# pfnet/sfm-learner-chainer

Hardware: AMD Instinct MI355X
Metric: warp+photo-loss fwd+bwd Mpixels/s @128x416x4scales; % HBM roofline (higher is better)
Workload: dtype f32

## Files before the change

### sfm-learner-chainer_amd/csrc/sfm_loss_kernels.h

```cpp
#pragma once
#include "sfm_common.h"
#include "sfm_ssim_pass.h"
#include "sfm_ssim_pair.h"

namespace sfm {

constexpr int MAX_CHUNK_ROWS = 28;
constexpr int MIN_CHUNK_ROWS = 4;
constexpr int WAVES_PER_BLOCK = 1;

struct ScaleArgs {
  const float* tgt;
  const float* src;
  const float* disp;
  const float* mlog;
  float* d_disp;
  float* d_mask;
  float* d_src;
  float* warped;
  int h, w, strips, chunks, tiles, item_begin, chunk_rows;
  float inv_cnt;
  float c_dx2, c_dy2, c_dxy;
  float c_ex, c_ey;
  float c_exp;
// ... 24 lines not shown
  Base = 0,
  Wide = 1,
  Pair = 2,
  Ref = 3,
  Dsrc = 4,
};
struct Variant {
  bool grad, loss;
  bool ssim, expl;
  int smode;
  bool hwc, warped;
  Family family;
};

struct HaloCols { int hs, hm, hr, hl, sw; };
constexpr HaloCols halo_of(const bool ssim, const bool grad, const int smode) {
  const int hs = ssim ? (grad ? 2 : 1) : 0;
  const int hm = smode == 1 ? 2 : (smode == 2 ? 1 : 0);
  const int hr = hs > hm ? hs : hm;
  const int hl = grad ? hr : hs;
  return {hs, hm, hr, hl, 64 - hl - hr};
}
constexpr HaloCols halo_of(const Variant& v) { return halo_of(v.ssim, v.grad, v.smode); }
template <bool SSIM, bool GRAD, int SMODE>
struct Halo {
  static constexpr int HS = halo_of(SSIM, GRAD, SMODE).hs, HR = halo_of(SSIM, GRAD, SMODE).hr, HL = halo_of(SSIM, GRAD, SMODE).hl,
                       SW = halo_of(SSIM, GRAD, SMODE).sw;
};
constexpr int waves_per_simd(const Family f, const bool ssim, const bool grad) {
  return f == Family::Pair ? 2 : (f == Family::Wide || (ssim && grad)) ? 3 : 4;
}
constexpr int waves_per_simd(const Variant& v) { return waves_per_simd(v.family, v.ssim, v.grad); }
constexpr int sources_per_pass(const Family f) { return f == Family::Pair ? 2 : 1; }

__device__ __forceinline__ void tile_put(float* p, const float v, const bool add) {
  if (add) *p = *p + v;
  else *p = v;
}

template <bool GRAD, bool LOSS>
__device__ __forceinline__ void smooth2_pass(const LossArgs& A, const ScaleArgs& S, const float* __restrict__ dplane, int lane,
                                             int x, bool xin, bool outl, int y0, int y1, float* gacc, float& acc_sm, const bool add) {
  const int h = S.h, w = S.w;
  const bool vx2 = xin && (x <= w - 3);
  const bool vx1 = xin && (x <= w - 2);
  const unsigned xc = (unsigned)min(max(x, 0), w - 1);
  auto ldrow = [&](int r) -> float { return ldf(dplane, (unsigned)min(max(r, 0), h - 1) * (unsigned)w + xc); };
  float c_dx2 = S.c_dx2, c_dy2 = S.c_dy2, c_dxy = S.c_dxy, gyv = A.gy;
  asm volatile("" : "+v"(c_dx2), "+v"(c_dy2), "+v"(c_dxy), "+v"(gyv));
  float s2y_m1 = 0.f, s2y_m2 = 0.f, txy_m1 = 0.f;
  auto row = [&](const int a, float& d0, float& dp1, float& q) {
    q = xin ? q : 0.f;
    const float dp2 = q;
    const float dxr0 = from_right(d0) - d0;
    const float dx2 = from_right(dxr0) - dxr0;
    const float dy0 = dp1 - d0, dy1 = dp2 - dp1;
    const float dy2 = dy1 - dy0;
    const float dxrp = from_right(dp1) - dp1;
    const float dxdy0 = dxrp - dxr0;
    const float dydx0 = from_right(dy0) - dy0;
    d0 = ldrow(a + 5);
    const bool va = a >= 0, va2 = va && a <= h - 3, va1 = va && a <= h - 2;
    if (LOSS) {
      if (a >= y0) {
        float t = 0.f;
        if (vx2) t += c_dx2 * fabsf(dx2);
// ... 209 lines not shown
  const int prio_rank = min((int)(blockIdx.x >> 3) / H.simds_per_xcd, H.prio_top);
  set_issue_prio((int)((H.prio_tab >> (2 * prio_rank)) & 3u));
  const int chunk = t / S.strips;
  const int strip = t - chunk * S.strips;
  const int h = S.h, w = S.w;
  const int lane = threadIdx.x & 63;
  const int x = strip * HH::SW - HH::HL + lane;
  const bool xin = (x >= 0) && (x < w);
  const bool outl = (lane >= HH::HL) && (lane < 64 - HH::HR) && (x < w);
  const int y0 = chunk * S.chunk_rows;
  const int y1 = min(y0 + S.chunk_rows, h);
  const ScaleConst sc = make_scale_const(h, w);
  const size_t P = (size_t)h * w;

  float acc_pix = 0.f, acc_ssim = 0.f, acc_sm = 0.f, acc_exp = 0.f;
  bool first = true;
  float disp_first, disp_second;
  {
    const float* dpl = S.disp + (size_t)b * P;
    const int rfirst = y0 - HH::HS;
    const unsigned xcl = (unsigned)min(max(x, 0), w - 1);
    disp_first = ldf(dpl, (unsigned)min(max(rfirst, 0), h - 1) * (unsigned)w + xcl);
    disp_second = ldf(dpl, (unsigned)min(max(rfirst + 1, 0), h - 1) * (unsigned)w + xcl);
  }
  static_assert(SFM_MAX_SRC * 8 <= 64, "one group of eight lanes per source");
  WaveGeom WG;
  WaveGeomRef WGR;
  build_wave_geom_any<REF != 0>(A.pose, H.n_src, b, A.intrinsics + (size_t)(b * H.n_scales + s) * 9, lane, WG, WGR);
#ifdef SFM_STAMPS
  Stamps st = {0, 0, 0, 0, 0};
  unsigned long long ts0 = 0, cyc_smooth = 0, cyc_src = 0;
  SFM_STAMP(ts0);
#endif
  const bool smooth_last = (SMODE != 0) && (prio_rank == 1);
  const int n_units = PAIR ? (H.n_src >> 1) : H.n_src;
  const int n_phases = n_units + (SMODE != 0 ? 1 : 0);
  for (int ph = 0; ph < n_phases; ++ph) {
    const int iu = (SMODE != 0 && !smooth_last) ? ph - 1 : ph;
    const int i = PAIR ? 2 * iu : iu;
#ifdef SFM_STAMPS
    unsigned long long tp0 = 0, tp1 = 0;
    SFM_STAMP(tp0);
#endif
    if (SMODE != 0 && (iu < 0 || iu >= n_units)) {
      if (SMODE == 1) smooth2_pass<GRAD, LOSS>(A, S, S.disp + (size_t)b * P, lane, x, xin, outl, y0, y1, gacc, acc_sm, !first);
      else smooth_edge_pass<GRAD, LOSS, HWC>(A, S, S.disp + (size_t)b * P, S.tgt + (size_t)b * 3 * P, lane, x, xin, outl, y0, y1, gacc, acc_sm, !first);
      first = false;
#ifdef SFM_STAMPS
      SFM_STAMP(tp1);
      cyc_smooth += tp1 - tp0;
#endif
      continue;
    }
    if (iu * 2 >= n_units) set_issue_prio((int)((H.prio_tab >> (8 + 2 * prio_rank)) & 3u));
    SsimCtx C;
    const float xf = (float)x;
    C.x0 = x - lane;
    if constexpr (REF != 0) {
#pragma unroll
      for (int k = 0; k < 3; ++k) {
        C.Pm[k * 4 + 0] = from_lane(WGR.P0, 8 * i + k);
        C.Pm[k * 4 + 1] = from_lane(WGR.P1, 8 * i + k);
        C.Pm[k * 4 + 2] = from_lane(WGR.P2, 8 * i + k);
        C.Pm[k * 4 + 3] = from_lane(WGR.P3, 8 * i + k);
        C.Ki1[k] = from_lane(WGR.Ki1, k);
        C.Ki2[k] = from_lane(WGR.Ki2, k);
        C.mx[k] = from_lane(WGR.Ki0, k) * xf;
        C.M1[k] = C.P3[k] = 0.f;
      }
#pragma unroll
      for (int k = 0; k < 3; ++k) C.P3[k] = C.Pm[k * 4 + 3];
      C.hw[0] = 0.5f * sc.wm1; C.hw[1] = 0.5f * sc.hm1;
      C.rhw[0] = uniform(rcp_refined(C.hw[0])); C.rhw[1] = uniform(rcp_refined(C.hw[1]));
    } else {
#pragma unroll
      for (int k = 0; k < 3; ++k) {
        C.M1[k] = from_lane(WG.M1, 8 * i + k);
        C.P3[k] = from_lane(WG.P3, 8 * i + k);
        C.mx[k] = fmaf(from_lane(WG.M0, 8 * i + k), xf, from_lane(WG.M2, 8 * i + k));
      }
    }
#pragma unroll
    for (int k = 0; k < 3; ++k) {
      C.tp[k] = S.tgt + ((size_t)b * 3 + k) * P;
      C.sp[k] = S.src + (((size_t)b * H.n_src + i) * 3 + k) * P;
    }
    C.k_pix = S.k_pix;
    C.kq = S.kq;
    C.k_exp = S.k_exp;
    int y0p = y0, y1p = y1;
    asm volatile("" : "+s"(y0p), "+s"(y1p));
    C.h = h; C.w = w; C.y0 = y0p; C.y1 = y1p;
    C.dp = S.disp + (size_t)b * P;
    C.dsp = (DSRC && S.d_src) ? S.d_src + ((size_t)b * H.n_src + i) * 3 * P : nullptr;
    C.wp = WARPED ? S.warped + ((size_t)b * H.n_src + i) * 3 * P : nullptr;
    C.mp = EXPL ? S.mlog + ((size_t)b * H.n_src + i) * P : nullptr;
    C.dmp = (EXPL && GRAD) ? S.d_mask + ((size_t)b * H.n_src + i) * P : nullptr;
    C.P = P;
    C.sc = sc;
    C.xc = (unsigned)min(max(x, 0), w - 1);
    C.disp_first = disp_first;
    C.disp_second = disp_second;
    C.xc12 = 12u * C.xc;
    C.x12 = 12u * (unsigned)x;
    C.img12 = 12u * (unsigned)h * (unsigned)w;
    C.w12 = 12u * (unsigned)w;
    C.w12f = (float)(12 * w);
    C.xin = xin;
    C.outb = outl;
    C.xinf = xin ? 1.f : 0.f;
    C.outf = outl ? 1.f : 0.f;
    C.lane = lane;
    float* gpm_out = GRAD ? A.part_gpm + ((size_t)item * H.n_src + i) * 12 : nullptr;
    if constexpr (PAIR) {
      SsimCtx Cb = C;
#pragma unroll
      for (int k = 0; k < 3; ++k) {
        Cb.M1[k] = from_lane(WG.M1, 8 * (i + 1) + k);
        Cb.P3[k] = from_lane(WG.P3, 8 * (i + 1) + k);
        Cb.mx[k] = fmaf(from_lane(WG.M0, 8 * (i + 1) + k), xf, from_lane(WG.M2, 8 * (i + 1) + k));
        Cb.sp[k] = C.sp[k] + 3 * P;
      }
      Cb.wp = WARPED ? C.wp + 3 * P : nullptr;
      ssim_pair_pass<GRAD, LOSS, WARPED>(C, Cb, gacc, first, acc_pix, acc_ssim, gpm_out, GRAD ? gpm_out + 12 : nullptr);
    } else if constexpr (SSIM) {
      ssim_source_pass<GRAD, LOSS, HWC, WARPED, REF, DSRC>(C, gacc, first, acc_pix, acc_ssim, gpm_out SFM_STAMPS_PASS);
    } else {
      l1_source_pass<GRAD, LOSS, EXPL, HWC, WARPED, REF, DSRC>(C, gacc, first, acc_pix, acc_exp, gpm_out);
    }
    first = false;
#ifdef SFM_STAMPS
    SFM_STAMP(tp1);
    cyc_src += tp1 - tp0;
#endif
  }
  if (LOSS) {
    float v[4] = {acc_pix, acc_ssim, acc_sm, acc_exp};
    wave_sums_lockstep(v);
    if (lane == 63) {
      float* o = A.part_loss + (size_t)item * 4;
      o[0] = v[0] * S.inv_cnt; o[1] = v[1] * S.inv_cnt; o[2] = v[2]; o[3] = v[3] * S.c_exp;
    }
  }
  if (GRAD) {
    if (outl) {
      float* o = S.d_disp + (size_t)b * P;
      for (int q = y0; q < y1; ++q) stf_wt(o, (unsigned)(q * w + x), gacc[(q - y0) * 64 + lane]);
    }
  }
  if (H.trace && lane == 0) {
    unsigned long long* o = H.trace + (size_t)item * 4;
    o[0] = t_start;
    o[1] = __builtin_amdgcn_s_memrealtime();
    o[2] = __builtin_amdgcn_s_getreg((4) | (0 << 6) | (31 << 11));
    o[3] = (__builtin_amdgcn_s_getreg((20) | (0 << 6) | (31 << 11)) & 0xf) | ((unsigned long long)blockIdx.x << 8);
#ifdef SFM_STAMPS
    {
      unsigned long long* q = H.trace + (size_t)H.items * 4 + (size_t)item * 8;
      unsigned long long ts3 = 0;
      SFM_STAMP(ts3);
      q[0] = st.a_fin; q[1] = st.a_iss; q[2] = st.b; q[3] = st.c; q[4] = st.steps > 0 ? st.steps : 1;
      q[5] = cyc_smooth;
      q[6] = cyc_src;
      q[7] = ts3 - ts0;
    }
#endif
  }
}

template <bool SSIM, bool GRAD, bool LOSS, bool EXPL, int SMODE, bool HWC, bool WARPED = false>
__global__ void __launch_bounds__(64 * WAVES_PER_BLOCK, waves_per_simd(Family::Base, SSIM, GRAD)) loss_kernel(SFM_HDR_PARAMS, const LossArgs A) {
  loss_body<SSIM, GRAD, LOSS, EXPL, SMODE, HWC, WARPED>(make_hdr(A, SFM_HDR_ARGS), A);
}
template <bool SSIM, bool LOSS, bool EXPL, int SMODE, bool HWC, bool WARPED = false>
__global__ void __launch_bounds__(64 * WAVES_PER_BLOCK, waves_per_simd(Family::Dsrc, SSIM, true)) loss_kernel_dsrc(SFM_HDR_PARAMS, const LossArgs A) {
  loss_body<SSIM, true, LOSS, EXPL, SMODE, HWC, WARPED, 0, true>(make_hdr(A, SFM_HDR_ARGS), A);
}
template <bool SSIM, bool GRAD, bool LOSS, bool EXPL, int SMODE, bool HWC, bool WARPED = false>
__global__ void __launch_bounds__(64 * WAVES_PER_BLOCK, waves_per_simd(Family::Ref, SSIM, GRAD)) loss_kernel_ref(SFM_HDR_PARAMS, const LossArgs A) {
  loss_body<SSIM, GRAD, LOSS, EXPL, SMODE, HWC, WARPED, 1, GRAD>(make_hdr(A, SFM_HDR_ARGS), A);
}
template <bool GRAD, bool LOSS, int SMODE>
__global__ void __launch_bounds__(64 * WAVES_PER_BLOCK, waves_per_simd(Family::Pair, true, GRAD)) loss_kernel_pair(SFM_HDR_PARAMS, const LossArgs A) {
  loss_body<true, GRAD, LOSS, false, SMODE, true, false, 0, false, true>(make_hdr(A, SFM_HDR_ARGS), A);
}
template <bool LOSS, int SMODE, bool HWC, bool WARPED = false>
__global__ void __launch_bounds__(64 * WAVES_PER_BLOCK, waves_per_simd(Family::Wide, false, true)) loss_kernel_wide(SFM_HDR_PARAMS, const LossArgs A) {
  loss_body<false, true, LOSS, false, SMODE, HWC, WARPED>(make_hdr(A, SFM_HDR_ARGS), A);
}

template <Family F, bool GRAD, bool LOSS, bool SSIM, bool EXPL, int SMODE, bool HWC, bool WARPED>
const void* family_kernel() {
  if constexpr (F == Family::Base) return (const void*)&loss_kernel<SSIM, GRAD, LOSS, EXPL, SMODE, HWC, WARPED>;
  else if constexpr (F == Family::Ref) return (const void*)&loss_kernel_ref<SSIM, GRAD, LOSS, EXPL, SMODE, HWC, WARPED>;
  else if constexpr (F == Family::Dsrc && GRAD) return (const void*)&loss_kernel_dsrc<SSIM, LOSS, EXPL, SMODE, HWC, WARPED>;
// ... 66 lines not shown
```

### sfm-learner-chainer_amd/csrc/sfm_ssim_pass.h

```cpp
#pragma once
#include "sfm_common.h"

namespace sfm {

#ifdef SFM_STAMPS
#define SFM_STAMP(var) do { __builtin_amdgcn_sched_barrier(0); asm volatile("s_memtime %0\n s_waitcnt lgkmcnt(0)" : "=s"(var) :: "memory"); __builtin_amdgcn_sched_barrier(0); } while (0)
struct Stamps { unsigned long long a_fin, a_iss, b, c, steps; };
static __device__ Stamps g_dummy_stamps;
#define SFM_STAMPS_ARG , Stamps& st
#define SFM_STAMPS_PASS , st
#else
#define SFM_STAMP(var) do { } while (0)
#define SFM_STAMPS_ARG
#define SFM_STAMPS_PASS
#endif

struct SsimCtx {
  float M1[3], P3[3];
  float Ki1[3], Ki2[3], Pm[12], hw[2], rhw[2];
  int x0;
  float k_pix;
  float kq;
  int h, w, y0, y1;
  const float* tp[3];
  const float* sp[3];
  const float* dp;
  float* dsp;
  float* wp;
  const float* mp;
  float* dmp;
  float k_exp;
  size_t P;
  ScaleConst sc;
  float mx[3];
  float disp_first, disp_second;
  unsigned xc;
  unsigned xc12;
  unsigned x12;
  unsigned img12;
  unsigned w12;
  float w12f;
  bool xin;
  bool outb;
  float xinf;
  float outf;
  int lane;
};

typedef float f2 __attribute__((ext_vector_type(2)));
struct Ch3 {
  f2 p;
  float s;
};
__device__ __forceinline__ Ch3 ch3(float c0, float c1, float c2) { Ch3 r; r.p.x = c0; r.p.y = c1; r.s = c2; return r; }
__device__ __forceinline__ Ch3 ch3_zero() { return ch3(0.f, 0.f, 0.f); }

template <typename T> __device__ __forceinline__ T T_of(float v);
template <> __device__ __forceinline__ float T_of<float>(float v) { return v; }
template <> __device__ __forceinline__ f2 T_of<f2>(float v) { f2 r; r.x = v; r.y = v; return r; }
__device__ __forceinline__ f2 vfma(f2 a, f2 b, f2 c) { return __builtin_elementwise_fma(a, b, c); }
__device__ __forceinline__ float vfma(float a, float b, float c) { return fmaf(a, b, c); }
__device__ __forceinline__ f2 vrcp(f2 a) { f2 r; r.x = rcp(a.x); r.y = rcp(a.y); return r; }
__device__ __forceinline__ float vrcp(float a) { return rcp(a); }
__device__ __forceinline__ f2 hsum3(f2 v) { f2 r; r.x = hsum3(v.x); r.y = hsum3(v.y); return r; }
// ... 30 lines not shown
}
__device__ __forceinline__ void hsum3_group(f2& a, f2& b, f2& c, float& e, float& f, float& g) {
  pin(a); pin(b); pin(c); pin(e); pin(f); pin(g);
  __builtin_amdgcn_sched_barrier(0);
  const float le = add_left(e), lf = add_left(f), lg = add_left(g);
  const f2 la = add_left(a), lb = add_left(b), lc = add_left(c);
  e = add_right(le, e); f = add_right(lf, f); g = add_right(lg, g);
  a = add_right(la, a); b = add_right(lb, b); c = add_right(lc, c);
  __builtin_amdgcn_sched_barrier(0);
}
__device__ __forceinline__ float half_one_minus_clamped(float S) { return fminf(fmaxf(fmaf(S, -0.5f, 0.5f), 0.f), 1.f); }
__device__ __forceinline__ f2 half_one_minus_clamped(f2 S) {
  f2 r;
  asm("v_pk_fma_f32 %0, %1, 0.5, 0.5 op_sel_hi:[1,0,0] neg_lo:[1,0,0] neg_hi:[1,0,0] clamp" : "=v"(r) : "v"(S));
  return r;
}
__device__ __forceinline__ float sign01(float d) {
  const float big = 0x1p127f;
  float sp, sm;
  asm("v_mul_f32_e64 %0, %1, %2 clamp" : "=v"(sp) : "v"(d), "s"(big));
  asm("v_mul_f32_e64 %0, -%1, %2 clamp" : "=v"(sm) : "v"(d), "s"(big));
  return sp - sm;
}
__device__ __forceinline__ f2 sign01(f2 d) {
  f2 big;
  big.x = 0x1p127f; big.y = 0x1p127f;
  f2 sp, sm;
  asm("v_pk_mul_f32 %0, %1, %2 clamp" : "=v"(sp) : "v"(d), "s"(big));
  asm("v_pk_mul_f32 %0, %1, %2 neg_lo:[1,0] neg_hi:[1,0] clamp" : "=v"(sm) : "v"(d), "s"(big));
  return sp - sm;
}
__device__ __forceinline__ float ksign(float k, float d) { return k * sign01(d); }
__device__ __forceinline__ f2 ksign(float k, f2 d) { return sign01(d) * k; }
__device__ __forceinline__ float add_ksign(float g, float k, float d) { return fmaf(sign01(d), k, g); }
__device__ __forceinline__ f2 add_ksign(f2 g, float k, f2 d) { return vfma(sign01(d), T_of<f2>(k), g); }
__device__ __forceinline__ float vabs_sum(f2 d) { return fabsf(d.x) + fabsf(d.y); }
__device__ __forceinline__ float vabs_sum(float d) { return fabsf(d); }
__device__ __forceinline__ float vhadd(f2 v) { return v.x + v.y; }
__device__ __forceinline__ float vhadd(float v) { return v; }

struct __attribute__((packed, aligned(4))) Rgb {
  float c[3];
};
__device__ __forceinline__ Rgb load_rgb(const float* p) { return *reinterpret_cast<const Rgb*>(p); }
struct __attribute__((packed, aligned(4))) K9 {
  float k[9];
};
__device__ __forceinline__ K9 load_k9(const float* Kp) { return *reinterpret_cast<const K9*>(Kp); }

__device__ __forceinline__ float from_lane(const float v, const int k) {
  return __builtin_bit_cast(float, __builtin_amdgcn_readlane(__builtin_bit_cast(int, v), k));
}
__device__ __forceinline__ float from_lane_v(const float v, const int src) {
  return __builtin_bit_cast(float, __builtin_amdgcn_ds_bpermute(src << 2, __builtin_bit_cast(int, v)));
}

__device__ __forceinline__ void inv3_fast(const float* K, float* o) {
  const float a = K[0], b = K[1], c = K[2], d = K[3], e = K[4], f = K[5], g = K[6], h = K[7], i = K[8];
  const float A = fmaf(e, i, -(f * h)), B = fmaf(f, g, -(d * i)), Cc = fmaf(d, h, -(e * g));
  const float det = fmaf(a, A, fmaf(b, B, c * Cc));
  const float r = rcp_refined(det);
  o[0] = A * r;
  o[1] = fmaf(c, h, -(b * i)) * r;
  o[2] = fmaf(b, f, -(c * e)) * r;
  o[3] = B * r;
  o[4] = fmaf(a, i, -(c * g)) * r;
// ... 102 lines not shown
  f2 duv0, duv1, duv_s;
  f2 UV;
  float D;
  float rzi;
  float nm;
};
struct RowG { Ch3 a, b, e; };

struct Pipe {
  float ta[3], tb[3];
  float ba[3], bb[3];
  float it[3];
  f2 UV, f;
  float rz, D;
  float lg;
  bool inview;
  bool inview_o;
};

__device__ __forceinline__ void zero(RowS& s) {
  s.ih = s.it = ch3_zero(); s.duv0 = s.duv1 = s.duv_s = T_of<f2>(0.f);
  s.UV = T_of<f2>(0.f); s.D = s.rzi = s.nm = 0.f;
}
__device__ __forceinline__ void zero(RowG& s) { s.a = s.b = s.e = ch3_zero(); }
__device__ __forceinline__ float opaque_zero() {
  float z;
  asm volatile("v_mov_b32 %0, 0" : "=v"(z));
  return z;
}
__device__ __forceinline__ Ch3 ch3_opaque_zero() {
  const float a = opaque_zero(), b = opaque_zero(), c = opaque_zero();
  return ch3(a, b, c);
}
__device__ __forceinline__ void zero_rare(RowS& s) {
  s.ih = ch3_opaque_zero(); s.it = ch3_opaque_zero();
  s.duv0.x = opaque_zero(); s.duv0.y = opaque_zero(); s.duv1.x = opaque_zero(); s.duv1.y = opaque_zero(); s.duv_s.x = opaque_zero(); s.duv_s.y = opaque_zero();
  s.UV.x = opaque_zero(); s.UV.y = opaque_zero(); s.D = opaque_zero(); s.rzi = opaque_zero(); s.nm = opaque_zero();
}

struct __attribute__((packed, aligned(4))) Rgb2 {
  float c[6];
};

struct RefPos {
  f2 UV;
  f2 fr, cell;
  float rz, D;
  bool inview;
};
__device__ __forceinline__ Proj ref_proj_cell(const RefPos& rp, const int h, const int w) {
  Proj p;
  p.U = rp.UV.x; p.V = rp.UV.y; p.rz = rp.rz; p.inview = rp.inview;
  int u0 = (int)rp.cell.x, v0 = (int)rp.cell.y;
  p.fu = rp.fr.x; p.fv = rp.fr.y;
  if (u0 > w - 2) { u0 = w - 2; p.fu = 1.f; }
  if (v0 > h - 2) { v0 = h - 2; p.fv = 1.f; }
  p.u0 = rp.inview ? u0 : 0;
  p.v0 = rp.inview ? v0 : 0;
  return p;
}
__device__ __forceinline__ RefPos ref_position(const SsimCtx& C, const float yf, const float D ) {
  RefPos o;
  o.D = D;
  f2 ray, q, kxp, Ki1p, Ki2p, Pc0, Pc1, Pc2, Pc3, hwp, rhwp, whm1;
  kxp.x = C.mx[0]; kxp.y = C.mx[1]; Ki1p.x = C.Ki1[0]; Ki1p.y = C.Ki1[1]; Ki2p.x = C.Ki2[0]; Ki2p.y = C.Ki2[1];
  Pc0.x = C.Pm[0]; Pc0.y = C.Pm[4]; Pc1.x = C.Pm[1]; Pc1.y = C.Pm[5]; Pc2.x = C.Pm[2]; Pc2.y = C.Pm[6]; Pc3.x = C.Pm[3]; Pc3.y = C.Pm[7];
  hwp.x = C.hw[0]; hwp.y = C.hw[1]; rhwp.x = C.rhw[0]; rhwp.y = C.rhw[1]; whm1.x = C.sc.wm1; whm1.y = C.sc.hm1;
  float q2;
  {
#pragma clang fp contract(off)
    ray = (kxp + Ki1p * yf) + Ki2p;
    const float ray2 = (C.mx[2] + C.Ki1[2] * yf) + C.Ki2[2];
    const f2 c = ray * o.D;
    const float c2 = ray2 * o.D;
    q = ((Pc0 * c.x + Pc1 * c.y) + Pc2 * c2) + Pc3;
    q2 = ((C.Pm[8] * c.x + C.Pm[9] * c.y) + C.Pm[10] * c2) + C.Pm[11];
  }
  const float z = q2 + 1e-10f;
  o.rz = rcp(z);
  const f2 qr = q * o.rz;
  o.UV = vfma(vfma(-qr, T_of<f2>(z), q), T_of<f2>(o.rz), qr);
  const f2 xr = o.UV * rhwp;
  const f2 xn = vfma(vfma(-xr, hwp, o.UV), rhwp, xr) - 1.0f;
  const f2 t = vfma(-xn, xn, T_of<f2>(1.0f));
  o.inview = (t.x > 0.0f) & (t.y > 0.0f);
  f2 up;
  {
#pragma clang fp contract(off)
    up = ((xn + 1.0f) * whm1) * 0.5f + 1.0f;
  }
  o.fr.x = __builtin_amdgcn_fractf(up.x); o.fr.y = __builtin_amdgcn_fractf(up.y);
  o.cell = (up - o.fr) - 1.0f;
  return o;
}

template <bool HWC, int REF = 0, bool SECOND = false>
__device__ __forceinline__ void issue_row(const SsimCtx& C, const int r, const float disp, Pipe& ps) {
  static_assert(!SECOND || (HWC && REF == 0), "two sources per pass: pixel-interleaved layout, the product's projection");
  const float yf = (float)r;
  Proj p;
  f2 UV, fr, cell;
  float rz;
  if constexpr (REF != 0) {
    const RefPos rp = ref_position(C, yf, rcp_refined(disp));
    ps.D = rp.D; UV = rp.UV; fr = rp.fr; cell = rp.cell; rz = rp.rz; p.inview = rp.inview;
    p.u0 = p.v0 = 0;
    if constexpr (!HWC) {
      p = ref_proj_cell(rp, C.h, C.w);
      fr.x = p.fu; fr.y = p.fv;
    }
  } else if constexpr (HWC) {
    if constexpr (!SECOND) ps.D = rcp(disp);
    f2 M1p, mxp, P3p, whm1;
    M1p.x = C.M1[0]; M1p.y = C.M1[1]; mxp.x = C.mx[0]; mxp.y = C.mx[1]; P3p.x = C.P3[0]; P3p.y = C.P3[1];
    whm1.x = C.sc.wm1; whm1.y = C.sc.hm1;
    const f2 a = vfma(M1p, T_of<f2>(yf), mxp);
    const float a2 = fmaf(C.M1[2], yf, C.mx[2]);
    const f2 q = vfma(T_of<f2>(ps.D), a, P3p);
    const float z = fmaf(ps.D, a2, C.P3[2]) + 1e-10f;
    rz = rcp(z);
    const f2 qr = q * rz;
    UV = vfma(vfma(-qr, T_of<f2>(z), q), T_of<f2>(rz), qr);
    const f2 sg = UV * (whm1 - UV);
    p.inview = (sg.x > 0.0f) & (sg.y > 0.0f);
    fr.x = __builtin_amdgcn_fractf(UV.x); fr.y = __builtin_amdgcn_fractf(UV.y);
    cell = UV - fr;
    p.u0 = p.v0 = 0;
  } else {
    ps.D = rcp(disp);
    const float a0 = fmaf(C.M1[0], yf, C.mx[0]), a1 = fmaf(C.M1[1], yf, C.mx[1]), a2 = fmaf(C.M1[2], yf, C.mx[2]);
    p = project(a0, a1, a2, C.P3[0], C.P3[1], C.P3[2], ps.D, C.sc, C.h, C.w);
    UV.x = p.U; UV.y = p.V; fr.x = p.fu; fr.y = p.fv; rz = p.rz;
    cell = UV;
  }
  ps.UV = UV; ps.f = fr;
  if constexpr (HWC) {
    ps.rz = (p.inview && C.outb) ? rz : 0.f;
    ps.inview = ps.inview_o = true;
  } else {
    ps.rz = rz;
    ps.inview = p.inview && C.xin;
    ps.inview_o = p.inview && C.outb;
  }
  const unsigned off = (unsigned)(p.v0 * C.w + p.u0);
  const unsigned offt = (unsigned)r * (unsigned)C.w + C.xc;
  if constexpr (HWC) {
    const float bof = fmaf(cell.y, C.w12f, cell.x * 12.f);
    const char* sp8 = reinterpret_cast<const char*>(C.sp[0]);
    const char* tp8 = reinterpret_cast<const char*>(C.tp[0]) + (size_t)((unsigned)r * C.w12);
    const __amdgpu_buffer_rsrc_t srs = __builtin_amdgcn_make_buffer_rsrc(const_cast<char*>(sp8), 0, (int)C.img12, 0x00027000);
    const __amdgpu_buffer_rsrc_t srs2 = __builtin_amdgcn_make_buffer_rsrc(const_cast<char*>(sp8 + C.w12), 0, (int)(C.img12 - C.w12), 0x00027000);
    const __amdgpu_buffer_rsrc_t trs = __builtin_amdgcn_make_buffer_rsrc(const_cast<char*>(tp8), 0, (int)C.w12, 0x00027000);
    const unsigned o12 = (p.inview && C.xin) ? (unsigned)bof : 0x80000000u;
    typedef unsigned u4v __attribute__((ext_vector_type(4)));
    typedef unsigned u3v __attribute__((ext_vector_type(3)));
    typedef unsigned u2v __attribute__((ext_vector_type(2)));
    const u4v t0 = __builtin_amdgcn_raw_buffer_load_b128(srs, o12, 0, 0);
    const u2v t1 = __builtin_amdgcn_raw_buffer_load_b64(srs, o12 + 16u, 0, 0);
    const u4v b0 = __builtin_amdgcn_raw_buffer_load_b128(srs2, o12, 0, 0);
    const u2v b1 = __builtin_amdgcn_raw_buffer_load_b64(srs2, o12 + 16u, 0, 0);
    u3v i0 = {0u, 0u, 0u};
    if constexpr (!SECOND) i0 = __builtin_amdgcn_raw_buffer_load_b96(trs, C.x12, 0, 0);
    Rgb2 T, Bt;
    Rgb I;
// ... 46 lines not shown
  }
}

__device__ __forceinline__ void store_warped_row(const SsimCtx& C, const int r, const RowS& s) {
  if ((unsigned)(r - C.y0) < (unsigned)(C.y1 - C.y0) && C.outb) {
    const unsigned o = (unsigned)r * (unsigned)C.w + C.xc;
    stf_wt(C.wp, o, s.ih.p.x);
    stf_wt(C.wp + C.P, o, s.ih.p.y);
    stf_wt(C.wp + 2 * C.P, o, s.ih.s);
  }
}

struct PoseAcc {
  f2 A, B, Cq;
  float A2, B2, C2;
};
__device__ __forceinline__ void zero(PoseAcc& a) {
  a.A = a.B = a.Cq = T_of<f2>(0.f); a.A2 = a.B2 = a.C2 = 0.f;
}


__device__ __forceinline__ float geom_terms(const SsimCtx& C, const f2 UV, const float D, const float yf, const f2 gq, PoseAcc& gpm) {
  const f2 guv = gq * UV;
  const float gq2 = -(guv.x + guv.y);
  const f2 t = gq * D;
  const float t2 = gq2 * D;
  const float gdisp = fmaf(t.x, C.P3[0], fmaf(t.y, C.P3[1], t2 * C.P3[2]));
  gpm.A += t; gpm.A2 += t2;
  gpm.B = vfma(T_of<f2>(yf), t, gpm.B); gpm.B2 = fmaf(yf, t2, gpm.B2);
  gpm.Cq += gq; gpm.C2 += gq2;
  return gdisp;
}

template <bool DSRC , int REF = 0>
__device__ __forceinline__ void geometry_backward(const SsimCtx& C, const RowS& s2, const int rc, const f2 gq,
                                                  const float* gI, float* gacc, const bool first, PoseAcc& gpm) {
  const int h = C.h, w = C.w;
  const float yf = (float)rc;
  const float gdisp = geom_terms(C, s2.UV, s2.D, yf, gq, gpm);
  float* ga = gacc + (rc - C.y0) * 64 + C.lane;
  if (first) *ga = gdisp;
  else *ga = *ga + gdisp;
  if (DSRC && C.dsp != nullptr && C.outb) {
    struct __attribute__((packed, aligned(4))) Rec { float c[3]; };
    const unsigned o = (unsigned)rc * (unsigned)w + (unsigned)(C.x0 + C.lane);
    Rec g; g.c[0] = gI[0]; g.c[1] = gI[1]; g.c[2] = gI[2];
    reinterpret_cast<Rec*>(C.dsp)[o] = g;
  }
  (void)h;
}

__device__ __forceinline__ void pose_sums_raw(const SsimCtx& C, const PoseAcc& pa, float* gpm_out) {
  const float acc[9] = {pa.A.x, pa.A.y, pa.A2, pa.B.x, pa.B.y, pa.B2, pa.Cq.x, pa.Cq.y, pa.C2};
  const float xf = (float)(C.x0 + C.lane);
  float v[12];
#pragma unroll
  for (int k = 0; k < 3; ++k) {
    v[k * 4 + 0] = xf * acc[k];
    v[k * 4 + 1] = acc[3 + k];
    v[k * 4 + 2] = acc[k];
    v[k * 4 + 3] = acc[6 + k];
  }
  wave_sums_lockstep(v);
  if (C.lane == 63) {
    float4* o = reinterpret_cast<float4*>(gpm_out);
    o[0] = make_float4(v[0], v[1], v[2], v[3]);
    o[1] = make_float4(v[4], v[5], v[6], v[7]);
    o[2] = make_float4(v[8], v[9], v[10], v[11]);
  }
}

template <typename T>
struct SsimSums { T Sx, Sy, Sqq, Sxy; };

template <typename T>
// ... 44 lines not shown
  g = add_ksign(vfma(vfma(it, Eq, -(ih * Bq)), T_of<T>(9.f), Aq), kpn, diff);
}

template <bool GRAD, bool LOSS>
__device__ __forceinline__ void ssim_stage_b_row(const SsimCtx& C, const RowS& s2, const RowS& s1, const RowS& s0, RowG& g0,
                                                 const bool count, float& acc_pix, float& acc_ssim) {
  float ssum = 0.f;
  const float kq2_nm = C.kq * s1.nm;
  SsimSums<f2> pp;
  SsimSums<float> ps;
  ssim_vsums(s2.ih.p, s1.ih.p, s0.ih.p, s2.it.p, s1.it.p, s0.it.p, pp);
  ssim_vsums(s2.ih.s, s1.ih.s, s0.ih.s, s2.it.s, s1.it.s, s0.it.s, ps);
  hsum3_group(pp.Sx, pp.Sy, pp.Sqq, pp.Sxy, ps.Sx, ps.Sy, ps.Sqq, ps.Sxy);
  ssim_value_partials<GRAD, LOSS, true>(pp, kq2_nm, g0.a.p, g0.b.p, g0.e.p, ssum);
  ssim_value_partials<GRAD, LOSS, false>(ps, kq2_nm, g0.a.s, g0.b.s, g0.e.s, ssum);
  if (GRAD) hsum3_group(g0.a.p, g0.b.p, g0.e.p, g0.a.s, g0.b.s, g0.e.s);
  if (LOSS) {
    const float wgt = count ? s1.nm * C.outf : 0.f;
    acc_ssim = fmaf(ssum, wgt, acc_ssim);
    if (!GRAD) {
      const float e1 = vabs_sum(s1.ih.p - s1.it.p) + vabs_sum(s1.ih.s - s1.it.s);
      acc_pix = fmaf(e1, wgt, acc_pix);
    }
  }
}

__device__ __forceinline__ f2 contract_uv(const RowS& s, const f2 gp, const float gs) {
  f2 hq = T_of<f2>(gp.x) * s.duv0;
  hq = vfma(T_of<f2>(gp.y), s.duv1, hq);
  hq = vfma(T_of<f2>(gs), s.duv_s, hq);
  return hq * s.rzi;
}

template <bool LOSS, bool DSRC, int REF = 0>
__device__ __forceinline__ void ssim_stage_c_row(const SsimCtx& C, const int rc, const RowS& s2, const RowG& g2, const RowG& g1,
                                                 const RowG& g0, float* gacc, const bool first, PoseAcc& gpm, float& acc_pix) {
  const float kpn = C.k_pix * s2.nm;
  f2 gp, dp;
  float gs, ds;
  ssim_stage_c(g2.a.p, g1.a.p, g0.a.p, g2.b.p, g1.b.p, g0.b.p, g2.e.p, g1.e.p, g0.e.p, s2.ih.p, s2.it.p, kpn, gp, dp);
  ssim_stage_c(g2.a.s, g1.a.s, g0.a.s, g2.b.s, g1.b.s, g0.b.s, g2.e.s, g1.e.s, g0.e.s, s2.ih.s, s2.it.s, kpn, gs, ds);
  if (LOSS) acc_pix = fmaf(vabs_sum(dp) + vabs_sum(ds), s2.nm * C.outf, acc_pix);
  const float gI[3] = {gp.x, gp.y, gs};
  geometry_backward<DSRC, REF>(C, s2, rc, contract_uv(s2, gp, gs), gI, gacc, first, gpm);
}

struct StepMasks {
  unsigned fin;
  unsigned iss;
  unsigned b;
  unsigned cnt;
  unsigned c;
};
__device__ __forceinline__ unsigned step_range(int lo, int hi) {
  lo = min(max(lo, 0), 32);
  hi = min(max(hi, lo), 32);
  const unsigned long long one = 1ull;
  return (unsigned)(((one << hi) - 1ull) & ~((one << lo) - 1ull));
}
__device__ __forceinline__ bool step_bit(const unsigned m, const int k) { return ((m >> k) & 1u) != 0u; }

template <bool GRAD, bool LOSS, bool HWC, bool WARPED, int REF, bool DSRC>
__device__ __forceinline__ void ssim_row_step(const SsimCtx& C, const StepMasks& M, const int k, const int r, Pipe& ps, float& disp_next,
                                              RowS& s0, const RowS& s1, const RowS& s2,
                                              RowG& g0, const RowG& g1, const RowG& g2, float* gacc, const bool first,
                                              float& acc_pix, float& acc_ssim, PoseAcc& gpm SFM_STAMPS_ARG) {
  const int w = C.w;
#ifdef SFM_STAMPS
  unsigned long long t0 = 0, t1 = 0, t2 = 0, t3 = 0, t4 = 0;
#endif
  SFM_STAMP(t0);
  finish_row<HWC>(C, ps, s0);
  if (!step_bit(M.fin, k)) zero_rare(s0);
  if constexpr (WARPED) store_warped_row(C, r, s0);
  SFM_STAMP(t1);
  if (step_bit(M.iss, k)) {
    issue_row<HWC, REF>(C, r + 1, disp_next, ps);
    disp_next = ldf(C.dp, (unsigned)min(r + 2, C.h - 1) * (unsigned)w + C.xc);
  }
  SFM_STAMP(t2);

  if (step_bit(M.b, k)) {
    ssim_stage_b_row<GRAD, LOSS>(C, s2, s1, s0, g0, step_bit(M.cnt, k), acc_pix, acc_ssim);
  }

  SFM_STAMP(t3);
  if (GRAD) {
    if (step_bit(M.c, k)) {
      ssim_stage_c_row<LOSS, DSRC, REF>(C, r - 2, s2, g2, g1, g0, gacc, first, gpm, acc_pix);
    }
  }
  SFM_STAMP(t4);
#ifdef SFM_STAMPS
  st.a_fin += t1 - t0; st.a_iss += t2 - t1; st.b += t3 - t2; st.c += t4 - t3; st.steps += 1;
#endif
}

template <bool GRAD, bool LOSS, bool HWC, bool WARPED, int REF = 0, bool DSRC = false>
__device__ __forceinline__ void ssim_source_pass(const SsimCtx& C, float* gacc, const bool first, float& acc_pix, float& acc_ssim,
                                                 float* gpm_out  SFM_STAMPS_ARG) {
  constexpr int HS = GRAD ? 2 : 1;
  const int rbeg = C.y0 - HS, rend = C.y1 + HS;
  const int rload = min(rend, C.h);
  PoseAcc gpm;
  zero(gpm);
  RowS S0, S1, S2;
  RowG G0, G1, G2;
  Pipe ps;
  float disp_next = 1.f;
  const int n = rend - rbeg, R = C.y1 - C.y0;
  StepMasks M;
  M.fin = step_range(-rbeg, C.h - rbeg);
  M.iss = step_range(-rbeg - 1, rload - rbeg - 1);
  M.b = step_range(HS + 1 - (GRAD ? 1 : 0), n);
  M.cnt = step_range(HS + 1, HS + 1 + R);
  M.c = step_range(HS + 2, HS + 2 + R);
  if (rbeg >= 0 && rbeg < C.h) issue_row<HWC, REF>(C, rbeg, C.disp_first, ps);
  disp_next = C.disp_second;
  for (int k = 0; k < n; k += 3) {
    const int r = rbeg + k;
    ssim_row_step<GRAD, LOSS, HWC, WARPED, REF, DSRC>(C, M, k, r, ps, disp_next, S0, S2, S1, G0, G2, G1, gacc, first, acc_pix, acc_ssim, gpm SFM_STAMPS_PASS);
    if (k + 1 < n)
      ssim_row_step<GRAD, LOSS, HWC, WARPED, REF, DSRC>(C, M, k + 1, r + 1, ps, disp_next, S1, S0, S2, G1, G0, G2, gacc, first, acc_pix, acc_ssim, gpm SFM_STAMPS_PASS);
    if (k + 2 < n)
      ssim_row_step<GRAD, LOSS, HWC, WARPED, REF, DSRC>(C, M, k + 2, r + 2, ps, disp_next, S2, S1, S0, G2, G1, G0, gacc, first, acc_pix, acc_ssim, gpm SFM_STAMPS_PASS);
  }
  if (GRAD) {
    pose_sums_raw(C, gpm, gpm_out);
  }
}

template <bool GRAD, bool LOSS, bool EXPL, bool HWC, bool WARPED, int REF = 0, bool DSRC = false>
__device__ __forceinline__ void l1_source_pass(const SsimCtx& C, float* gacc, const bool first, float& acc_pix, float& acc_exp,
                                               float* gpm_out) {
  PoseAcc gpm;
  zero(gpm);
  Pipe ps;
  ps.lg = 0.f;
  float disp_next = 1.f;
  const int rbeg = C.y0, rend = C.y1;
  issue_row<HWC, REF>(C, rbeg, C.disp_first, ps);
  if (rbeg + 1 < rend) disp_next = C.disp_second;
  for (int r = rbeg; r < rend; ++r) {
    RowS s0;
    finish_row<HWC>(C, ps, s0);
    if constexpr (WARPED) store_warped_row(C, r, s0);
    const float lg = ps.lg;
    if (r + 1 < rend) issue_row<HWC, REF>(C, r + 1, disp_next, ps);
    disp_next = ldf(C.dp, (unsigned)min(r + 2, C.h - 1) * (unsigned)C.w + C.xc);
    float sgm = 1.f;
    if (EXPL) {
      sgm = rcp(1.0f + __expf(-lg));
      if (LOSS) acc_exp += C.outf * (fmaxf(-lg, 0.f) + __logf(1.0f + __expf(-fabsf(lg))));
    }
    const float e1 = (vabs_sum(s0.ih.p - s0.it.p) + vabs_sum(s0.ih.s - s0.it.s)) * s0.nm;
    if (LOSS) acc_pix = fmaf(e1 * sgm, C.outf, acc_pix);
    if (GRAD) {
      const float kpn = C.k_pix * s0.nm * sgm;
// ... 16 lines not shown
```

Before: 80990.

## Fuse edge-aware smoothness pass into the first or last SSIM source pass

When SSIM with edge-aware smoothness is active (non-pair, not ref-grad), the separate smoothness phase is removed. The smoothness loss and gradient are computed inside an SSIM source pass, reusing the target rows and disparity already loaded there. On the last source, the disparity gradient is combined with the pending geometry gradient before being stored. This removes one full pass over the disparity and target planes per tile. In exchange, the fused variant keeps raw disparity in the row state and recomputes its reciprocal in the backward step, which adds register pressure and arithmetic.

Result: slower. 78650 (-2.9%).

```diff
diff --git a/sfm-learner-chainer_amd/csrc/sfm_loss_kernels.h b/sfm-learner-chainer_amd/csrc/sfm_loss_kernels.h
--- a/sfm-learner-chainer_amd/csrc/sfm_loss_kernels.h
+++ b/sfm-learner-chainer_amd/csrc/sfm_loss_kernels.h
@@ -80,6 +80,7 @@
 }
 constexpr int waves_per_simd(const Variant& v) { return waves_per_simd(v.family, v.ssim, v.grad); }
 constexpr int sources_per_pass(const Family f) { return f == Family::Pair ? 2 : 1; }
+constexpr bool fuse_smooth(const bool ssim, const int smode, const bool pair, const bool ref_grad) { return ssim && smode == 2 && !pair && !ref_grad; }
 
 __device__ __forceinline__ void tile_put(float* p, const float v, const bool add) {
   if (add) *p = *p + v;
@@ -355,17 +356,18 @@
   unsigned long long ts0 = 0, cyc_smooth = 0, cyc_src = 0;
   SFM_STAMP(ts0);
 #endif
+  constexpr bool FUSED = fuse_smooth(SSIM, SMODE, PAIR, REF != 0 && GRAD);
   const bool smooth_last = (SMODE != 0) && (prio_rank == 1);
   const int n_units = PAIR ? (H.n_src >> 1) : H.n_src;
-  const int n_phases = n_units + (SMODE != 0 ? 1 : 0);
+  const int n_phases = n_units + ((SMODE != 0 && !FUSED) ? 1 : 0);
   for (int ph = 0; ph < n_phases; ++ph) {
-    const int iu = (SMODE != 0 && !smooth_last) ? ph - 1 : ph;
+    const int iu = (SMODE != 0 && !FUSED && !smooth_last) ? ph - 1 : ph;
     const int i = PAIR ? 2 * iu : iu;
 #ifdef SFM_STAMPS
     unsigned long long tp0 = 0, tp1 = 0;
     SFM_STAMP(tp0);
 #endif
-    if (SMODE != 0 && (iu < 0 || iu >= n_units)) {
+    if (SMODE != 0 && !FUSED && (iu < 0 || iu >= n_units)) {
       if (SMODE == 1) smooth2_pass<GRAD, LOSS>(A, S, S.disp + (size_t)b * P, lane, x, xin, outl, y0, y1, gacc, acc_sm, !first);
       else smooth_edge_pass<GRAD, LOSS, HWC>(A, S, S.disp + (size_t)b * P, S.tgt + (size_t)b * 3 * P, lane, x, xin, outl, y0, y1, gacc, acc_sm, !first);
       first = false;
@@ -411,6 +413,10 @@
     C.k_pix = S.k_pix;
     C.kq = S.kq;
     C.k_exp = S.k_exp;
+    if constexpr (FUSED) {
+      C.cex = S.c_ex; C.cey = S.c_ey;
+      C.gcx = uniform(A.gy * S.c_ex); C.gcy = uniform(A.gy * S.c_ey);
+    }
     int y0p = y0, y1p = y1;
     asm volatile("" : "+s"(y0p), "+s"(y1p));
     C.h = h; C.w = w; C.y0 = y0p; C.y1 = y1p;
@@ -446,8 +452,16 @@
       }
       Cb.wp = WARPED ? C.wp + 3 * P : nullptr;
       ssim_pair_pass<GRAD, LOSS, WARPED>(C, Cb, gacc, first, acc_pix, acc_ssim, gpm_out, GRAD ? gpm_out + 12 : nullptr);
+    } else if constexpr (FUSED) {
+      if (GRAD && smooth_last) {
+        if (iu == n_units - 1) ssim_source_pass<GRAD, LOSS, HWC, WARPED, REF, DSRC, GRAD ? 2 : 1, true>(C, gacc, first, acc_pix, acc_ssim, acc_sm, gpm_out SFM_STAMPS_PASS);
+        else ssim_source_pass<GRAD, LOSS, HWC, WARPED, REF, DSRC, 0, true>(C, gacc, first, acc_pix, acc_ssim, acc_sm, gpm_out SFM_STAMPS_PASS);
+      } else {
+        if (iu == 0) ssim_source_pass<GRAD, LOSS, HWC, WARPED, REF, DSRC, 1, true>(C, gacc, first, acc_pix, acc_ssim, acc_sm, gpm_out SFM_STAMPS_PASS);
+        else ssim_source_pass<GRAD, LOSS, HWC, WARPED, REF, DSRC, 0, true>(C, gacc, first, acc_pix, acc_ssim, acc_sm, gpm_out SFM_STAMPS_PASS);
+      }
     } else if constexpr (SSIM) {
-      ssim_source_pass<GRAD, LOSS, HWC, WARPED, REF, DSRC>(C, gacc, first, acc_pix, acc_ssim, gpm_out SFM_STAMPS_PASS);
+      ssim_source_pass<GRAD, LOSS, HWC, WARPED, REF, DSRC>(C, gacc, first, acc_pix, acc_ssim, acc_sm, gpm_out SFM_STAMPS_PASS);
     } else {
       l1_source_pass<GRAD, LOSS, EXPL, HWC, WARPED, REF, DSRC>(C, gacc, first, acc_pix, acc_exp, gpm_out);
     }
@@ -483,7 +497,7 @@
       unsigned long long ts3 = 0;
       SFM_STAMP(ts3);
       q[0] = st.a_fin; q[1] = st.a_iss; q[2] = st.b; q[3] = st.c; q[4] = st.steps > 0 ? st.steps : 1;
-      q[5] = cyc_smooth;
+      q[5] = FUSED ? (1ull << 63) | st.sm : cyc_smooth;
       q[6] = cyc_src;
       q[7] = ts3 - ts0;
     }
diff --git a/sfm-learner-chainer_amd/csrc/sfm_ssim_pass.h b/sfm-learner-chainer_amd/csrc/sfm_ssim_pass.h
--- a/sfm-learner-chainer_amd/csrc/sfm_ssim_pass.h
+++ b/sfm-learner-chainer_amd/csrc/sfm_ssim_pass.h
@@ -5,7 +5,7 @@
 
 #ifdef SFM_STAMPS
 #define SFM_STAMP(var) do { __builtin_amdgcn_sched_barrier(0); asm volatile("s_memtime %0\n s_waitcnt lgkmcnt(0)" : "=s"(var) :: "memory"); __builtin_amdgcn_sched_barrier(0); } while (0)
-struct Stamps { unsigned long long a_fin, a_iss, b, c, steps; };
+struct Stamps { unsigned long long a_fin, a_iss, b, c, steps, sm; };
 static __device__ Stamps g_dummy_stamps;
 #define SFM_STAMPS_ARG , Stamps& st
 #define SFM_STAMPS_PASS , st
@@ -30,6 +30,7 @@
   const float* mp;
   float* dmp;
   float k_exp;
+  float cex, cey, gcx, gcy;
   size_t P;
   ScaleConst sc;
   float mx[3];
@@ -126,6 +127,7 @@
 }
 __device__ __forceinline__ float ksign(float k, float d) { return k * sign01(d); }
 __device__ __forceinline__ f2 ksign(float k, f2 d) { return sign01(d) * k; }
+__device__ __forceinline__ float ksign_med3(float k, float d) { return k * __builtin_amdgcn_fmed3f(d * 0x1p127f, -1.f, 1.f); }
 __device__ __forceinline__ float add_ksign(float g, float k, float d) { return fmaf(sign01(d), k, g); }
 __device__ __forceinline__ f2 add_ksign(f2 g, float k, f2 d) { return vfma(sign01(d), T_of<f2>(k), g); }
 __device__ __forceinline__ float vabs_sum(f2 d) { return fabsf(d.x) + fabsf(d.y); }
@@ -294,10 +296,12 @@
   const float a = opaque_zero(), b = opaque_zero(), c = opaque_zero();
   return ch3(a, b, c);
 }
+template <bool KEEP_D = false>
 __device__ __forceinline__ void zero_rare(RowS& s) {
   s.ih = ch3_opaque_zero(); s.it = ch3_opaque_zero();
   s.duv0.x = opaque_zero(); s.duv0.y = opaque_zero(); s.duv1.x = opaque_zero(); s.duv1.y = opaque_zero(); s.duv_s.x = opaque_zero(); s.duv_s.y = opaque_zero();
-  s.UV.x = opaque_zero(); s.UV.y = opaque_zero(); s.D = opaque_zero(); s.rzi = opaque_zero(); s.nm = opaque_zero();
+  s.UV.x = opaque_zero(); s.UV.y = opaque_zero(); s.rzi = opaque_zero(); s.nm = opaque_zero();
+  if constexpr (!KEEP_D) s.D = opaque_zero();
 }
 
 struct __attribute__((packed, aligned(4))) Rgb2 {
@@ -356,30 +360,32 @@
   return o;
 }
 
-template <bool HWC, int REF = 0, bool SECOND = false>
+template <bool HWC, int REF = 0, bool SECOND = false, bool DRAW = false>
 __device__ __forceinline__ void issue_row(const SsimCtx& C, const int r, const float disp, Pipe& ps) {
   static_assert(!SECOND || (HWC && REF == 0), "two sources per pass: pixel-interleaved layout, the product's projection");
+  static_assert(!SECOND || !DRAW, "two sources per pass keep their own smoothness pass");
   const float yf = (float)r;
   Proj p;
   f2 UV, fr, cell;
   float rz;
   if constexpr (REF != 0) {
     const RefPos rp = ref_position(C, yf, rcp_refined(disp));
-    ps.D = rp.D; UV = rp.UV; fr = rp.fr; cell = rp.cell; rz = rp.rz; p.inview = rp.inview;
+    ps.D = DRAW ? disp : rp.D; UV = rp.UV; fr = rp.fr; cell = rp.cell; rz = rp.rz; p.inview = rp.inview;
     p.u0 = p.v0 = 0;
     if constexpr (!HWC) {
       p = ref_proj_cell(rp, C.h, C.w);
       fr.x = p.fu; fr.y = p.fv;
     }
   } else if constexpr (HWC) {
-    if constexpr (!SECOND) ps.D = rcp(disp);
+    float Dv = ps.D;
+    if constexpr (!SECOND) Dv = rcp(disp);
     f2 M1p, mxp, P3p, whm1;
     M1p.x = C.M1[0]; M1p.y = C.M1[1]; mxp.x = C.mx[0]; mxp.y = C.mx[1]; P3p.x = C.P3[0]; P3p.y = C.P3[1];
     whm1.x = C.sc.wm1; whm1.y = C.sc.hm1;
     const f2 a = vfma(M1p, T_of<f2>(yf), mxp);
     const float a2 = fmaf(C.M1[2], yf, C.mx[2]);
-    const f2 q = vfma(T_of<f2>(ps.D), a, P3p);
-    const float z = fmaf(ps.D, a2, C.P3[2]) + 1e-10f;
+    const f2 q = vfma(T_of<f2>(Dv), a, P3p);
+    const float z = fmaf(Dv, a2, C.P3[2]) + 1e-10f;
     rz = rcp(z);
     const f2 qr = q * rz;
     UV = vfma(vfma(-qr, T_of<f2>(z), q), T_of<f2>(rz), qr);
@@ -388,10 +394,12 @@
     fr.x = __builtin_amdgcn_fractf(UV.x); fr.y = __builtin_amdgcn_fractf(UV.y);
     cell = UV - fr;
     p.u0 = p.v0 = 0;
+    if constexpr (!SECOND) ps.D = DRAW ? disp : Dv;
   } else {
-    ps.D = rcp(disp);
+    const float Dv = rcp(disp);
+    ps.D = DRAW ? disp : Dv;
     const float a0 = fmaf(C.M1[0], yf, C.mx[0]), a1 = fmaf(C.M1[1], yf, C.mx[1]), a2 = fmaf(C.M1[2], yf, C.mx[2]);
-    p = project(a0, a1, a2, C.P3[0], C.P3[1], C.P3[2], ps.D, C.sc, C.h, C.w);
+    p = project(a0, a1, a2, C.P3[0], C.P3[1], C.P3[2], Dv, C.sc, C.h, C.w);
     UV.x = p.U; UV.y = p.V; fr.x = p.fu; fr.y = p.fv; rz = p.rz;
     cell = UV;
   }
@@ -504,15 +512,23 @@
   return gdisp;
 }
 
-template <bool DSRC , int REF = 0>
+template <bool DSRC , int REF = 0, int SMV = 0>
 __device__ __forceinline__ void geometry_backward(const SsimCtx& C, const RowS& s2, const int rc, const f2 gq,
-                                                  const float* gI, float* gacc, const bool first, PoseAcc& gpm) {
+                                                  const float* gI, float* gacc, const bool first, PoseAcc& gpm, float* pend = nullptr) {
   const int h = C.h, w = C.w;
   const float yf = (float)rc;
-  const float gdisp = geom_terms(C, s2.UV, s2.D, yf, gq, gpm);
+  const float D = (SMV == 0) ? s2.D : (REF != 0) ? rcp_refined(s2.D) : rcp(s2.D);
+  const float gdisp = geom_terms(C, s2.UV, D, yf, gq, gpm);
   float* ga = gacc + (rc - C.y0) * 64 + C.lane;
-  if (first) *ga = gdisp;
-  else *ga = *ga + gdisp;
+  if constexpr (SMV == 1) {
+    *ga = *ga + gdisp;
+  } else if constexpr (SMV == 2) {
+    if (first) *pend = gdisp;
+    else *pend = *ga + gdisp;
+  } else {
+    if (first) *ga = gdisp;
+    else *ga = *ga + gdisp;
+  }
   if (DSRC && C.dsp != nullptr && C.outb) {
     struct __attribute__((packed, aligned(4))) Rec { float c[3]; };
     const unsigned o = (unsigned)rc * (unsigned)w + (unsigned)(C.x0 + C.lane);
@@ -623,9 +639,10 @@
   return hq * s.rzi;
 }
 
-template <bool LOSS, bool DSRC, int REF = 0>
+template <bool LOSS, bool DSRC, int REF = 0, int SMV = 0>
 __device__ __forceinline__ void ssim_stage_c_row(const SsimCtx& C, const int rc, const RowS& s2, const RowG& g2, const RowG& g1,
-                                                 const RowG& g0, float* gacc, const bool first, PoseAcc& gpm, float& acc_pix) {
+                                                 const RowG& g0, float* gacc, const bool first, PoseAcc& gpm, float& acc_pix,
+                                                 float* pend = nullptr) {
   const float kpn = C.k_pix * s2.nm;
   f2 gp, dp;
   float gs, ds;
@@ -633,7 +650,31 @@
   ssim_stage_c(g2.a.s, g1.a.s, g0.a.s, g2.b.s, g1.b.s, g0.b.s, g2.e.s, g1.e.s, g0.e.s, s2.ih.s, s2.it.s, kpn, gs, ds);
   if (LOSS) acc_pix = fmaf(vabs_sum(dp) + vabs_sum(ds), s2.nm * C.outf, acc_pix);
   const float gI[3] = {gp.x, gp.y, gs};
-  geometry_backward<DSRC, REF>(C, s2, rc, contract_uv(s2, gp, gs), gI, gacc, first, gpm);
+  geometry_backward<DSRC, REF, SMV>(C, s2, rc, contract_uv(s2, gp, gs), gI, gacc, first, gpm, pend);
+}
+
+template <bool GRAD, bool LOSS, int SMV>
+__device__ __forceinline__ void smooth_edge_row(const SsimCtx& C, const RowS& c0, const RowS& c1, const int q,
+                                                const bool count, float* gacc, const float pend, float& sy_prev, float& acc_sm) {
+  const float KE = -1.44269504088896341f / 3.0f;
+  const float sx = ((from_right(c0.it.p.x) - c0.it.p.x) + (from_right(c0.it.p.y) - c0.it.p.y)) + (from_right(c0.it.s) - c0.it.s);
+  const float sy3 = ((c1.it.p.x - c0.it.p.x) + (c1.it.p.y - c0.it.p.y)) + (c1.it.s - c0.it.s);
+  const float ddx = from_right(c0.D) - c0.D;
+  const float ddy = c1.D - c0.D;
+  float wx;
+  asm("v_cmp_gt_u32_e32 vcc, %2, %3\n\tv_cndmask_b32_e32 %0, 0, %1, vcc" : "=v"(wx) : "v"(__builtin_amdgcn_exp2f(fabsf(sx) * KE)), "s"(C.w12 - 12u), "v"(C.x12) : "vcc");
+  const float wy = __builtin_amdgcn_exp2f(fabsf(sy3) * KE);
+  const float sy = ksign_med3(wy, ddy);
+  const float tx = ksign_med3(wx, ddx);
+  const float gx = from_left(tx) - tx;
+  if (count) {
+    if (LOSS) acc_sm = fmaf(C.outf, fmaf(C.cex * fabsf(ddx), wx, C.cey * fabsf(ddy) * wy), acc_sm);
+    if (GRAD) {
+      const float g = fmaf(C.gcy, sy_prev - sy, C.gcx * gx);
+      gacc[(q - C.y0) * 64 + C.lane] = (SMV == 2) ? pend + g : g;
+    }
+  }
+  sy_prev = sy;
 }
 
 struct StepMasks {
@@ -642,6 +683,7 @@
   unsigned b;
   unsigned cnt;
   unsigned c;
+  unsigned sm;
 };
 __device__ __forceinline__ unsigned step_range(int lo, int hi) {
   lo = min(max(lo, 0), 32);
@@ -651,22 +693,22 @@
 }
 __device__ __forceinline__ bool step_bit(const unsigned m, const int k) { return ((m >> k) & 1u) != 0u; }
 
-template <bool GRAD, bool LOSS, bool HWC, bool WARPED, int REF, bool DSRC>
+template <bool GRAD, bool LOSS, bool HWC, bool WARPED, int REF, bool DSRC, int SMV>
 __device__ __forceinline__ void ssim_row_step(const SsimCtx& C, const StepMasks& M, const int k, const int r, Pipe& ps, float& disp_next,
                                               RowS& s0, const RowS& s1, const RowS& s2,
                                               RowG& g0, const RowG& g1, const RowG& g2, float* gacc, const bool first,
-                                              float& acc_pix, float& acc_ssim, PoseAcc& gpm SFM_STAMPS_ARG) {
+                                              float& acc_pix, float& acc_ssim, float& acc_sm, float& sy_prev, PoseAcc& gpm SFM_STAMPS_ARG) {
   const int w = C.w;
 #ifdef SFM_STAMPS
-  unsigned long long t0 = 0, t1 = 0, t2 = 0, t3 = 0, t4 = 0;
+  unsigned long long t0 = 0, t1 = 0, t2 = 0, t3 = 0, t3s = 0, t4 = 0;
 #endif
   SFM_STAMP(t0);
   finish_row<HWC>(C, ps, s0);
-  if (!step_bit(M.fin, k)) zero_rare(s0);
+  if (!step_bit(M.fin, k)) zero_rare<SMV != 0>(s0);
   if constexpr (WARPED) store_warped_row(C, r, s0);
   SFM_STAMP(t1);
   if (step_bit(M.iss, k)) {
-    issue_row<HWC, REF>(C, r + 1, disp_next, ps);
+    issue_row<HWC, REF, false, SMV != 0>(C, r + 1, disp_next, ps);
     disp_next = ldf(C.dp, (unsigned)min(r + 2, C.h - 1) * (unsigned)w + C.xc);
   }
   SFM_STAMP(t2);
@@ -676,20 +718,29 @@
   }
 
   SFM_STAMP(t3);
+  float pend = 0.f;
   if (GRAD) {
     if (step_bit(M.c, k)) {
-      ssim_stage_c_row<LOSS, DSRC, REF>(C, r - 2, s2, g2, g1, g0, gacc, first, gpm, acc_pix);
+      ssim_stage_c_row<LOSS, DSRC, REF, SMV>(C, r - 2, s2, g2, g1, g0, gacc, first, gpm, acc_pix, &pend);
+    }
+  }
+  SFM_STAMP(t3s);
+  if constexpr (SMV != 0) {
+    if (step_bit(M.sm, k)) {
+      if constexpr (SMV == 1) smooth_edge_row<GRAD, LOSS, 1>(C, s1, s0, r - 1, step_bit(M.cnt, k), gacc, 0.f, sy_prev, acc_sm);
+      else smooth_edge_row<GRAD, LOSS, 2>(C, s2, s1, r - 2, step_bit(M.c, k), gacc, pend, sy_prev, acc_sm);
     }
   }
   SFM_STAMP(t4);
 #ifdef SFM_STAMPS
-  st.a_fin += t1 - t0; st.a_iss += t2 - t1; st.b += t3 - t2; st.c += t4 - t3; st.steps += 1;
+  st.a_fin += t1 - t0; st.a_iss += t2 - t1; st.b += t3 - t2; st.c += t3s - t3; st.sm += t4 - t3s; st.steps += 1;
 #endif
 }
 
-template <bool GRAD, bool LOSS, bool HWC, bool WARPED, int REF = 0, bool DSRC = false>
+template <bool GRAD, bool LOSS, bool HWC, bool WARPED, int REF = 0, bool DSRC = false, int SMV = 0, bool OWN2 = false>
 __device__ __forceinline__ void ssim_source_pass(const SsimCtx& C, float* gacc, const bool first, float& acc_pix, float& acc_ssim,
-                                                 float* gpm_out  SFM_STAMPS_ARG) {
+                                                 float& acc_sm, float* gpm_out  SFM_STAMPS_ARG) {
+  static_assert(GRAD || SMV != 2, "forward only: there is no tile, the term rides on the first pass");
   constexpr int HS = GRAD ? 2 : 1;
   const int rbeg = C.y0 - HS, rend = C.y1 + HS;
   const int rload = min(rend, C.h);
@@ -706,15 +757,18 @@
   M.b = step_range(HS + 1 - (GRAD ? 1 : 0), n);
   M.cnt = step_range(HS + 1, HS + 1 + R);
   M.c = step_range(HS + 2, HS + 2 + R);
-  if (rbeg >= 0 && rbeg < C.h) issue_row<HWC, REF>(C, rbeg, C.disp_first, ps);
-  disp_next = C.disp_second;
+  M.sm = (SMV == 0) ? 0u : step_range(HS + SMV - ((GRAD && C.y0 > 0) ? 1 : 0), HS + SMV + R);
+  float sy_prev = 0.f;
+  if (rbeg >= 0 && rbeg < C.h) issue_row<HWC, REF, false, SMV != 0>(C, rbeg, C.disp_first, ps);
+  if constexpr (OWN2) disp_next = ldf(C.dp, (unsigned)min(max(rbeg + 1, 0), C.h - 1) * (unsigned)C.w + C.xc);
+  else disp_next = C.disp_second;
   for (int k = 0; k < n; k += 3) {
     const int r = rbeg + k;
-    ssim_row_step<GRAD, LOSS, HWC, WARPED, REF, DSRC>(C, M, k, r, ps, disp_next, S0, S2, S1, G0, G2, G1, gacc, first, acc_pix, acc_ssim, gpm SFM_STAMPS_PASS);
+    ssim_row_step<GRAD, LOSS, HWC, WARPED, REF, DSRC, SMV>(C, M, k, r, ps, disp_next, S0, S2, S1, G0, G2, G1, gacc, first, acc_pix, acc_ssim, acc_sm, sy_prev, gpm SFM_STAMPS_PASS);
     if (k + 1 < n)
-      ssim_row_step<GRAD, LOSS, HWC, WARPED, REF, DSRC>(C, M, k + 1, r + 1, ps, disp_next, S1, S0, S2, G1, G0, G2, gacc, first, acc_pix, acc_ssim, gpm SFM_STAMPS_PASS);
+      ssim_row_step<GRAD, LOSS, HWC, WARPED, REF, DSRC, SMV>(C, M, k + 1, r + 1, ps, disp_next, S1, S0, S2, G1, G0, G2, gacc, first, acc_pix, acc_ssim, acc_sm, sy_prev, gpm SFM_STAMPS_PASS);
     if (k + 2 < n)
-      ssim_row_step<GRAD, LOSS, HWC, WARPED, REF, DSRC>(C, M, k + 2, r + 2, ps, disp_next, S2, S1, S0, G2, G1, G0, gacc, first, acc_pix, acc_ssim, gpm SFM_STAMPS_PASS);
+      ssim_row_step<GRAD, LOSS, HWC, WARPED, REF, DSRC, SMV>(C, M, k + 2, r + 2, ps, disp_next, S2, S1, S0, G2, G1, G0, gacc, first, acc_pix, acc_ssim, acc_sm, sy_prev, gpm SFM_STAMPS_PASS);
   }
   if (GRAD) {
     pose_sums_raw(C, gpm, gpm_out);
```
